# prismformore/Multi-Task-Transformer

Measured on AMD Instinct MI355X. Metric: training images/sec (512x512, 6 tasks), higher is better.
Workload: dtype f32(bf16x3)

## Files before the change

multi-task-transformer_amd/csrc/attn_fast.hip:

```cpp
#include "mtt_device.h"
#include <type_traits>

namespace {

constexpr int KV = 64, HD = 64;
constexpr int KTILE = KV * HD * 2;
constexpr float LOG2E = 1.4426950408889634f;

struct AttnP { mtt_attn_desc d; };

__device__ __attribute__((aligned(32))) const unsigned g_attn_zero_page[8] = {0u, 0u, 0u, 0u, 0u, 0u, 0u, 0u};
MTT_DEV void attn_glds16(const bf16_t* src, unsigned char* lds_wave_base) {
  __builtin_amdgcn_global_load_lds((const __attribute__((address_space(1))) void*)src,
                                   (__attribute__((address_space(3))) void*)lds_wave_base, 16, 0, 0);
}
MTT_DEV bool attn_block_dead(const mtt_attn_desc& d, int b, int qb) {
  return d.skip_scale != nullptr && qb * 128 >= d.T && d.skip_scale[2 * b + 1] == 0.0f;
}
MTT_DEV void attn_store_dead_block(const mtt_attn_desc& d, int b, int h, int qb) {
  const int N = d.N, C = d.nH * HD, tid = threadIdx.x;
  const u32x4 z = (u32x4){0u, 0u, 0u, 0u};
#pragma unroll
  for (int i = 0; i < 4; ++i) {
    const int idx = tid + 256 * i, qrow = qb * 128 + (idx >> 3);
    if (qrow >= N) continue;
    const int64_t oi = ((int64_t)b * N + qrow) * C + h * HD + (idx & 7) * 8;
    *(u32x4*)((bf16_t*)d.out + oi) = z;
    if (d.out_lo) *(u32x4*)((bf16_t*)d.out_lo + oi) = z;
  }
  if (d.lse && tid < 128 && qb * 128 + tid < N) d.lse[((int64_t)b * d.nH + h) * N + qb * 128 + tid] = 0.f;
}
template <int OFF>
MTT_DEV u32x2 attn_ds_read_tr16(unsigned addr) {
  u32x2 r;
  asm volatile("ds_read_b64_tr_b16 %0, %1 offset:%2" : "=v"(r) : "v"(addr), "n"(OFF) : "memory");
  return r;
}
__global__ __launch_bounds__(256, 2) void attn_fwd_fast_kernel(const AttnP p) {
  extern __shared__ __attribute__((aligned(16))) unsigned char smem[];
  constexpr int STAGE = 2 * KTILE;
  const mtt_attn_desc& d = p.d;
  const int nqb = (d.N + 127) / 128;
  const int wi = xcd_remap(blockIdx.x, gridDim.x);
  const int qb = wi % nqb, bh = wi / nqb;
  const int h = bh % d.nH, b = bh / d.nH;
  if (attn_block_dead(d, b, qb)) { attn_store_dead_block(d, b, h, qb); return; }
  const int N = d.N, C = d.nH * HD;
  const int tid = threadIdx.x, lane = tid & 63, wave = tid >> 6;
  const int li = lane & 15, lg = lane >> 4;
  const int64_t tok0 = (int64_t)b * N;
  const bf16_t* qkv = (const bf16_t*)d.qkv;
  const int q0 = qb * 128 + wave * 32;
  const bool active = q0 < N;

  u32x4 qf[2][2], dummy;
#pragma unroll
  for (int sub = 0; sub < 2; ++sub) {
    const int qrow = q0 + sub * 16 + li;
    const bool ok = qrow < N;
#pragma unroll
    for (int kh = 0; kh < 2; ++kh) {
      Raw8<false> r;
// ... 186 lines not shown
    if (qrow >= N) continue;
    const float inv = 1.0f / l;
#pragma unroll
    for (int dt = 0; dt < 4; ++dt)
      *(u32x2*)(out + (tok0 + qrow) * C + h * HD + dt * 16 + lg * 4) =
          (u32x2){pack2(o[sub][dt][0] * inv, o[sub][dt][1] * inv), pack2(o[sub][dt][2] * inv, o[sub][dt][3] * inv)};
    if (d.lse && lg == 0) d.lse[((int64_t)b * d.nH + h) * N + qrow] = (m_run[sub] + log2f(l)) * 0.6931471805599453f;
  }
}


__global__ __launch_bounds__(256, 2) void attn_fwd_x3_kernel(const AttnP p) {
  extern __shared__ __attribute__((aligned(16))) unsigned char smem[];
  constexpr int STAGE = 4 * KTILE;
  const mtt_attn_desc& d = p.d;
  const int nqb = (d.N + 127) / 128;
  const int wi = xcd_remap(blockIdx.x, gridDim.x);
  const int qb = wi % nqb, bh = wi / nqb;
  const int h = bh % d.nH, b = bh / d.nH;
  if (attn_block_dead(d, b, qb)) { attn_store_dead_block(d, b, h, qb); return; }
  const int N = d.N, C = d.nH * HD;
  const int tid = threadIdx.x, lane = tid & 63, wave = tid >> 6;
  const int li = lane & 15, lg = lane >> 4;
  const int64_t tok0 = (int64_t)b * N;
  const bf16_t* qh_ = (const bf16_t*)d.qkv;
  const bf16_t* ql_ = (const bf16_t*)d.qkv_lo;
  const int q0 = qb * 128 + wave * 32;
  const bool active = q0 < N;

  u32x4 qfh[2][2], qfl[2][2];
#pragma unroll
  for (int sub = 0; sub < 2; ++sub) {
    const int qrow = q0 + sub * 16 + li;
    const bool ok = qrow < N;
    const int64_t qi = (tok0 + (ok ? qrow : 0)) * 3 * C + h * HD + lg * 8;
#pragma unroll
    for (int kh = 0; kh < 2; ++kh) {
      const u32x4 z = (u32x4){0u, 0u, 0u, 0u};
      qfh[sub][kh] = ok ? *(const u32x4*)(qh_ + qi + kh * 32) : z;
      qfl[sub][kh] = ok ? *(const u32x4*)(ql_ + qi + kh * 32) : z;
    }
  }

  int dma_off[4], dma_row[2];
  uint64_t zpage = (uint64_t)(uintptr_t)g_attn_zero_page;
  asm volatile("" : "+s"(zpage));
#pragma unroll
  for (int i = 0; i < 2; ++i) {
    const int r = wave * 16 + i * 8 + (lane >> 3), pc = lane & 7;
    dma_row[i] = r;
    dma_off[i] = r * 3 * C + C + ((pc ^ (r >> 1)) & 7) * 8;
    dma_off[2 + i] = r * 3 * C + 2 * C + (((((pc >> 1) ^ (r >> 1)) & 3) << 1) | (pc & 1)) * 8;
  }
  auto dma_issue = [&](unsigned char* st, int kv0) {
    const int64_t boff = (tok0 + kv0) * 3 * C + h * HD;
    const bool full = kv0 + KV <= N;
#pragma unroll
    for (int pl = 0; pl < 2; ++pl) {
      const bf16_t* base = (pl ? ql_ : qh_) + boff;
#pragma unroll
      for (int kv = 0; kv < 2; ++kv) {
        unsigned char* dst = st + (kv * 2 + pl) * KTILE + wave * 2048;
#pragma unroll
        for (int i = 0; i < 2; ++i) {
          const bool ok = full || kv0 + dma_row[i] < N;
          attn_glds16((const bf16_t*)(uintptr_t)(ok ? (uint64_t)(uintptr_t)(base + dma_off[kv * 2 + i]) : zpage), dst + i * 1024);
        }
      }
    }
  };
  const int vrow = 4 * lg + (li >> 2);
  const int vf_ = (vrow >> 1) & 3;
  unsigned vaddr[4];
#pragma unroll
  for (int dt = 0; dt < 4; ++dt) vaddr[dt] = (unsigned)(uintptr_t)smem + (unsigned)(2 * KTILE + vrow * 128 + (li & 3) * 8 + ((dt ^ vf_) & 3) * 32);
  const unsigned char* kaddr[2];
#pragma unroll
  for (int kh = 0; kh < 2; ++kh) kaddr[kh] = smem + li * 128 + (((kh * 4 + lg) ^ (li >> 1)) & 7) * 16;

  f32x4 o[2][4];
#pragma unroll
  for (int sub = 0; sub < 2; ++sub)
#pragma unroll
    for (int t = 0; t < 4; ++t) o[sub][t] = (f32x4){0.f, 0.f, 0.f, 0.f};
  float m_run[2] = {-INFINITY, -INFINITY}, l_part[2] = {0.f, 0.f};
  const float sc2 = d.scale * LOG2E;
  const bool write_raw = d.rawlog != nullptr && d.T > 0 && qb == 0 && wave == 0 && li < d.T;

  const int nkv = (N + KV - 1) / KV;
  dma_issue(smem, 0);
  asm volatile("s_waitcnt vmcnt(0)" ::: "memory");
  __syncthreads();

  auto tile = [&](auto stage_tag, int j) {
    constexpr int ST = decltype(stage_tag)::value;
    const bool more = j + 1 < nkv;
    if (more) dma_issue(smem + (1 - ST) * STAGE, (j + 1) * KV);
    const int kv0 = j * KV;
    if (active) {
      f32x4 s[2][4];
      {
        u32x4 kf[4][2];
#pragma unroll
        for (int kt = 0; kt < 4; ++kt)
#pragma unroll
          for (int kh = 0; kh < 2; ++kh) kf[kt][kh] = *(const u32x4*)(kaddr[kh] + ST * STAGE + kt * 2048);
        __builtin_amdgcn_s_setprio(1);
#pragma unroll
        for (int kt = 0; kt < 4; ++kt) {
          s[0][kt] = (f32x4){0.f, 0.f, 0.f, 0.f};
          s[1][kt] = (f32x4){0.f, 0.f, 0.f, 0.f};
#pragma unroll
          for (int kh = 0; kh < 2; ++kh) {
            s[0][kt] = mfma16(kf[kt][kh], qfl[0][kh], s[0][kt]);
            s[1][kt] = mfma16(kf[kt][kh], qfl[1][kh], s[1][kt]);
            s[0][kt] = mfma16(kf[kt][kh], qfh[0][kh], s[0][kt]);
            s[1][kt] = mfma16(kf[kt][kh], qfh[1][kh], s[1][kt]);
          }
        }
        __builtin_amdgcn_s_setprio(0);
#pragma unroll
        for (int kt = 0; kt < 4; ++kt)
#pragma unroll
          for (int kh = 0; kh < 2; ++kh) kf[kt][kh] = *(const u32x4*)(kaddr[kh] + ST * STAGE + KTILE + kt * 2048);
        __builtin_amdgcn_s_setprio(1);
#pragma unroll
        for (int kt = 0; kt < 4; ++kt)
#pragma unroll
          for (int kh = 0; kh < 2; ++kh) {
            s[0][kt] = mfma16(kf[kt][kh], qfh[0][kh], s[0][kt]);
            s[1][kt] = mfma16(kf[kt][kh], qfh[1][kh], s[1][kt]);
          }
        __builtin_amdgcn_s_setprio(0);
      }
      if (write_raw) {
        float* rl = d.rawlog + (((int64_t)b * d.nH + h) * d.T + li) * N;
#pragma unroll
        for (int kt = 0; kt < 4; ++kt)
#pragma unroll
          for (int r = 0; r < 4; ++r) {
            const int key = kv0 + kt * 16 + lg * 4 + r;
            if (key < N) rl[key] = s[0][kt][r];
          }
      }
      if (kv0 + KV > N) {
#pragma unroll
        for (int sub = 0; sub < 2; ++sub)
#pragma unroll
          for (int kt = 0; kt < 4; ++kt)
#pragma unroll
            for (int r = 0; r < 4; ++r)
              if ((kv0 + kt * 16 + lg * 4 + r) >= N) s[sub][kt][r] = -INFINITY;
      }
      u32x4 pbh[2][2], pbl[2][2];
#pragma unroll
      for (int sub = 0; sub < 2; ++sub) {
        float mx = s[sub][0][0];
#pragma unroll
        for (int kt = 0; kt < 4; ++kt)
#pragma unroll
          for (int r = 0; r < 4; ++r) mx = fmaxf(mx, s[sub][kt][r]);
        mx = groups_max(mx);
        const float m_new = fmaxf(m_run[sub], mx * sc2);
        if (__builtin_amdgcn_ballot_w64(m_new != m_run[sub]) != 0) {
          const float alpha = __builtin_amdgcn_exp2f(m_run[sub] - m_new);
          l_part[sub] *= alpha;
#pragma unroll
          for (int t = 0; t < 4; ++t)
#pragma unroll
            for (int r = 0; r < 4; ++r) o[sub][t][r] *= alpha;
          m_run[sub] = m_new;
        }
        float rs = 0.f;
#pragma unroll
        for (int kt = 0; kt < 4; ++kt)
#pragma unroll
          for (int r = 0; r < 4; ++r) {
            const float pv = __builtin_amdgcn_exp2f(fmaf(s[sub][kt][r], sc2, -m_new));
            s[sub][kt][r] = pv;
            rs += pv;
          }
        l_part[sub] += rs;
#pragma unroll
        for (int ks = 0; ks < 2; ++ks) {
          const u32x4 ph = (u32x4){pack2(s[sub][2 * ks][0], s[sub][2 * ks][1]), pack2(s[sub][2 * ks][2], s[sub][2 * ks][3]),
                                   pack2(s[sub][2 * ks + 1][0], s[sub][2 * ks + 1][1]), pack2(s[sub][2 * ks + 1][2], s[sub][2 * ks + 1][3])};
          pbh[sub][ks] = ph;
          pbl[sub][ks] = (u32x4){pack2(s[sub][2 * ks][0] - lo_of(ph.x), s[sub][2 * ks][1] - hi_of(ph.x)),
                                 pack2(s[sub][2 * ks][2] - lo_of(ph.y), s[sub][2 * ks][3] - hi_of(ph.y)),
                                 pack2(s[sub][2 * ks + 1][0] - lo_of(ph.z), s[sub][2 * ks + 1][1] - hi_of(ph.z)),
                                 pack2(s[sub][2 * ks + 1][2] - lo_of(ph.w), s[sub][2 * ks + 1][3] - hi_of(ph.w))};
        }
      }
      const bool half1 = kv0 + 32 < N;
#define ATW(x) "+v"(x)
#pragma unroll
      for (int pass = 0; pass < 2; ++pass) {
        u32x2 v0l[4], v0h[4], v1l[4], v1h[4];
#pragma unroll
        for (int dt = 0; dt < 4; ++dt) {
          if (pass == 0) {
            v0l[dt] = attn_ds_read_tr16<ST * STAGE>(vaddr[dt]);
            v0h[dt] = attn_ds_read_tr16<ST * STAGE + 16 * 128>(vaddr[dt]);
          } else {
            v0l[dt] = attn_ds_read_tr16<ST * STAGE + KTILE>(vaddr[dt]);
            v0h[dt] = attn_ds_read_tr16<ST * STAGE + KTILE + 16 * 128>(vaddr[dt]);
          }
        }
#pragma unroll
        for (int dt = 0; dt < 4; ++dt) {
          if (pass == 0) {
            v1l[dt] = attn_ds_read_tr16<ST * STAGE + 32 * 128>(vaddr[dt]);
            v1h[dt] = attn_ds_read_tr16<ST * STAGE + 48 * 128>(vaddr[dt]);
          } else {
            v1l[dt] = attn_ds_read_tr16<ST * STAGE + KTILE + 32 * 128>(vaddr[dt]);
            v1h[dt] = attn_ds_read_tr16<ST * STAGE + KTILE + 48 * 128>(vaddr[dt]);
          }
        }
        asm volatile("s_waitcnt lgkmcnt(8)"
                     : ATW(v0l[0]), ATW(v0l[1]), ATW(v0l[2]), ATW(v0l[3]), ATW(v0h[0]), ATW(v0h[1]), ATW(v0h[2]), ATW(v0h[3]),
                       ATW(v1l[0]), ATW(v1l[1]), ATW(v1l[2]), ATW(v1l[3]), ATW(v1h[0]), ATW(v1h[1]), ATW(v1h[2]), ATW(v1h[3]) :: "memory");
        __builtin_amdgcn_s_setprio(1);
#pragma unroll
        for (int dt = 0; dt < 4; ++dt) {
          const u32x4 vf = (u32x4){v0l[dt][0], v0l[dt][1], v0h[dt][0], v0h[dt][1]};
          if (pass == 0) {
            o[0][dt] = mfma16(vf, pbl[0][0], o[0][dt]);
            o[1][dt] = mfma16(vf, pbl[1][0], o[1][dt]);
          }
          o[0][dt] = mfma16(vf, pbh[0][0], o[0][dt]);
          o[1][dt] = mfma16(vf, pbh[1][0], o[1][dt]);
        }
        asm volatile("s_waitcnt lgkmcnt(0)" : ATW(v1l[0]), ATW(v1l[1]), ATW(v1l[2]), ATW(v1l[3]), ATW(v1h[0]), ATW(v1h[1]), ATW(v1h[2]), ATW(v1h[3]) :: "memory");
        if (half1) {
#pragma unroll
          for (int dt = 0; dt < 4; ++dt) {
            const u32x4 vf = (u32x4){v1l[dt][0], v1l[dt][1], v1h[dt][0], v1h[dt][1]};
            if (pass == 0) {
              o[0][dt] = mfma16(vf, pbl[0][1], o[0][dt]);
              o[1][dt] = mfma16(vf, pbl[1][1], o[1][dt]);
            }
            o[0][dt] = mfma16(vf, pbh[0][1], o[0][dt]);
            o[1][dt] = mfma16(vf, pbh[1][1], o[1][dt]);
          }
        }
        __builtin_amdgcn_s_setprio(0);
      }
#undef ATW
    }
    if (more) asm volatile("s_waitcnt vmcnt(0)" ::: "memory");
    __syncthreads();
  };
  for (int j = 0; j < nkv; j += 2) {
    tile(std::integral_constant<int, 0>{}, j);
    if (j + 1 < nkv) tile(std::integral_constant<int, 1>{}, j + 1);
  }

  bf16_t* outh = (bf16_t*)d.out;
  bf16_t* outl = (bf16_t*)d.out_lo;
#pragma unroll
  for (int sub = 0; sub < 2; ++sub) {
    const float l = groups_sum(l_part[sub]);
    const int qrow = q0 + sub * 16 + li;
    if (qrow >= N) continue;
    const float inv = 1.0f / l;
#pragma unroll
    for (int dt = 0; dt < 4; ++dt) {
      const float v0 = o[sub][dt][0] * inv, v1 = o[sub][dt][1] * inv, v2 = o[sub][dt][2] * inv, v3 = o[sub][dt][3] * inv;
      const u32x2 hi = (u32x2){pack2(v0, v1), pack2(v2, v3)};
      const int64_t oi = (tok0 + qrow) * C + h * HD + dt * 16 + lg * 4;
      *(u32x2*)(outh + oi) = hi;
      *(u32x2*)(outl + oi) = (u32x2){pack2(v0 - lo_of(hi.x), v1 - hi_of(hi.x)), pack2(v2 - lo_of(hi.y), v3 - hi_of(hi.y))};
    }
    if (d.lse && lg == 0) d.lse[((int64_t)b * d.nH + h) * N + qrow] = (m_run[sub] + log2f(l)) * 0.6931471805599453f;
  }
}

}

int mtt_attn_fwd_x3_split(const mtt_attn_desc* dd, hipStream_t s) {
  constexpr int smem = 2 * 4 * KTILE;
  static std::atomic<unsigned long long> done{0};
  if (int e = mtt_ensure_dyn_lds((const void*)attn_fwd_x3_kernel, smem, done)) return e;
  AttnP p; p.d = *dd;
  dim3 grid((unsigned)(((dd->N + 127) / 128) * dd->nH * dd->B));
  hipLaunchKernelGGL(attn_fwd_x3_kernel, grid, dim3(256), smem, s, p);
  return (int)hipGetLastError();
}

int mtt_attn_fwd_fast(const mtt_attn_desc* dd, hipStream_t s) {
  constexpr int smem = 2 * 2 * KTILE;
  AttnP p; p.d = *dd;
  dim3 grid((unsigned)(((dd->N + 127) / 128) * dd->nH * dd->B));
  hipLaunchKernelGGL(attn_fwd_fast_kernel, grid, dim3(256), smem, s, p);
  return (int)hipGetLastError();
}
```

multi-task-transformer_amd/csrc/gemm.hip:

```cpp
#include "mtt_device.h"
#include <type_traits>

namespace {

#ifndef MTT_GROUP_M
#define MTT_GROUP_M 4
#endif
#ifndef MTT_RING
#define MTT_RING 1
#endif
constexpr int BM = 128, BN = 128, BK = 64;
constexpr int TILE_BYTES = BM * BK * 2;

struct GemmP {
  mtt_gemm_desc d;
  FastDiv divW, divH, divCp, div3;
  FastDiv divAmb, divDmb, divRmb;
  FastDiv divPsW, divPsH, divPsCo;
  FastDiv divSkip;
  int tiles_m, tiles_n;
  int group_m;
#ifdef MTT_GEMM_TRACE
  unsigned long long* trace;
#endif
};

#ifdef MTT_GEMM_TRACE
MTT_DEV unsigned long long trace_hwid() {
  unsigned a, b;
  asm volatile("s_getreg_b32 %0, hwreg(HW_REG_HW_ID)" : "=s"(a));
  asm volatile("s_getreg_b32 %0, hwreg(HW_REG_XCC_ID)" : "=s"(b));
  return (unsigned long long)a | ((unsigned long long)b << 32);
}
#define MTT_TRACE(slot) do { if (p.trace && threadIdx.x == 0) p.trace[(size_t)(blockIdx.x + gridDim.x * blockIdx.z) * 8 + (slot)] = __builtin_amdgcn_s_memtime(); } while (0)
#define MTT_TRACE_RT(slot) do { if (p.trace && threadIdx.x == 0) p.trace[(size_t)(blockIdx.x + gridDim.x * blockIdx.z) * 8 + (slot)] = __builtin_amdgcn_s_memrealtime(); } while (0)
#define MTT_TRACE_ID(tile) do { if (p.trace && threadIdx.x == 0) { p.trace[(size_t)(blockIdx.x + gridDim.x * blockIdx.z) * 8 + 6] = trace_hwid(); p.trace[(size_t)(blockIdx.x + gridDim.x * blockIdx.z) * 8 + 7] = (tile); } } while (0)
#else
#define MTT_TRACE(slot) do {} while (0)
#define MTT_TRACE_RT(slot) do {} while (0)
#define MTT_TRACE_ID(tile) do {} while (0)
#endif

MTT_DEV int64_t row_off(uint32_t m, int mb, int64_t bs, int64_t ld, FastDiv f) {
  if (mb <= 0) return (int64_t)m * ld;
  const uint32_t q = fdiv(m, f);
  return (int64_t)q * bs + (int64_t)(m - q * (uint32_t)mb) * ld;
}

MTT_DEV bool skip_rows_dead(const GemmP& p, uint32_t r0, uint32_t r1) {
  const uint32_t mb = (uint32_t)p.d.skip_mb, np = (uint32_t)p.d.skip_prompt;
  uint32_t q = fdiv(r0, p.divSkip);
  uint32_t o = r0 - q * mb;
  for (uint32_t r = r0; r < r1;) {
    const uint32_t c = o >= np ? 1u : 0u;
    if (p.d.skip_scale[2 * q + c] != 0.0f) return false;
    if (c) { r += mb - o; ++q; o = 0; }
    else { r += np - o; o = np; if (np == mb) { ++q; o = 0; } }
  }
  return true;
}


__device__ __attribute__((aligned(32))) const unsigned g_zero_page[8] = {0u, 0u, 0u, 0u, 0u, 0u, 0u, 0u};

template <bool X3, bool CONV, bool F32>
struct StagerK {
  const void* base; int dtype; int K; int c;
  int64_t roff[4]; bool rok[4];
  uint64_t zpage;
  unsigned tapmask[4];
  int tap, ci, knext;
  Raw8<F32> raw[4];

  MTT_DEV void init(const GemmP& p, const void* b, int dt, int row0, int rows, int64_t ld, int mb, int64_t bs, FastDiv fmb) {
// ... 1443 lines not shown

  for (int kt = 0; kt < nk; ++kt) {
    const unsigned st = (unsigned)((kt & 1) * STAGE);
#pragma unroll
    for (int kh = 0; kh < 2; ++kh) {
      if (kh == 0 && kt + 1 < nk) issue((kt + 1) & 1, kt + 1);
      const unsigned off = st + (unsigned)(kh * 32 * 512);
      u32x2 bl[NT], bh[NT], al[MT], ah[MT];
#pragma unroll
      for (int t = 0; t < NT; ++t) { bl[t] = ds_read_tr16(b_addr[t] + off); bh[t] = ds_read_tr16(b_addr[t] + off + 4 * 512); }
#pragma unroll
      for (int t = 0; t < MT; ++t) { al[t] = ds_read_tr16(a_addr[t] + off); ah[t] = ds_read_tr16(a_addr[t] + off + 4 * 512); }
#define TNW(x) "+v"(x)
#define TNW_A TNW(al[0]), TNW(al[1]), TNW(al[2]), TNW(al[3]), TNW(al[4]), TNW(al[5]), TNW(al[6]), TNW(al[7]), \
              TNW(ah[0]), TNW(ah[1]), TNW(ah[2]), TNW(ah[3]), TNW(ah[4]), TNW(ah[5]), TNW(ah[6]), TNW(ah[7])
      if constexpr (MEDGE) {
        if (kh == 1) asm volatile("s_waitcnt vmcnt(0) lgkmcnt(0)" : TNW(bl[0]), TNW(bl[1]), TNW(bh[0]), TNW(bh[1]), TNW_A :: "memory");
        else asm volatile("s_waitcnt lgkmcnt(0)" : TNW(bl[0]), TNW(bl[1]), TNW(bh[0]), TNW(bh[1]), TNW_A :: "memory");
      } else {
        if (kh == 1)
          asm volatile("s_waitcnt vmcnt(0) lgkmcnt(0)"
                       : TNW(bl[0]), TNW(bl[1]), TNW(bl[2]), TNW(bl[3]), TNW(bh[0]), TNW(bh[1]), TNW(bh[2]), TNW(bh[3]), TNW_A :: "memory");
        else
          asm volatile("s_waitcnt lgkmcnt(0)"
                       : TNW(bl[0]), TNW(bl[1]), TNW(bl[2]), TNW(bl[3]), TNW(bh[0]), TNW(bh[1]), TNW(bh[2]), TNW(bh[3]), TNW_A :: "memory");
      }
#undef TNW_A
#undef TNW
      u32x4 fa[MT], fb[NT];
#pragma unroll
      for (int t = 0; t < NT; ++t) fb[t] = (u32x4){bl[t][0], bl[t][1], bh[t][0], bh[t][1]};
#pragma unroll
      for (int t = 0; t < MT; ++t) fa[t] = (u32x4){al[t][0], al[t][1], ah[t][0], ah[t][1]};
      __builtin_amdgcn_sched_barrier(0);
      __builtin_amdgcn_s_barrier();
      __builtin_amdgcn_sched_barrier(0);
      __builtin_amdgcn_s_setprio(1);
#pragma unroll
      for (int a = 0; a < MT; ++a)
#pragma unroll
        for (int b = 0; b < NT; ++b) acc[a][b] = mfma16(fa[a], fb[b], acc[a][b]);
      __builtin_amdgcn_s_setprio(0);
      __builtin_amdgcn_sched_barrier(0);
      __builtin_amdgcn_s_barrier();
      __builtin_amdgcn_sched_barrier(0);
    }
  }
  if (!late) __builtin_amdgcn_s_barrier();
  __syncthreads();
  if constexpr (MEDGE) gemm_epilogue<256, WAVES_M, WAVES_N, MT, NT>(p, acc, smem, m0, n0, zo, zi);
  else gemm_epilogue_auto<256, WAVES_M, WAVES_N, MT, NT>(p, acc, smem, m0, n0, zo, zi);
}

template <bool CONVB>
__global__ __launch_bounds__(512, 1) void gemm_tn_kernel(const GemmP p) {
  extern __shared__ __attribute__((aligned(16))) unsigned char smem[];
  const int wg = xcd_remap(blockIdx.x, gridDim.x);
  const int tiles_n = (p.d.N + 255) / 256, tiles_m = (p.d.M + 255) / 256;
  int tile_m, tile_n;
  grouped_tile(wg, tiles_m, tiles_n, p.group_m, tile_m, tile_n);
  const int m0 = tile_m * 256, n0 = tile_n * 256;
  const int z = blockIdx.z;
  const int zo = z / p.d.batch_inner, zi = z - zo * p.d.batch_inner;
  if (MTT_R3_EDGE && p.d.M - m0 <= 128 && !p.d.colsum_out && p.d.store_mode == MTT_STORE_ROWS) tn_tile<CONVB, true>(p, smem, m0, n0, zo, zi);
  else tn_tile<CONVB, false>(p, smem, m0, n0, zo, zi);
}

template <bool CONVB>
int launch_tn(const GemmP& p, hipStream_t stream) {
  constexpr int smem = 2 * 2 * BK * 256 * 2;
  static std::atomic<unsigned long long> done{0};
  if (int e = mtt_ensure_dyn_lds((const void*)gemm_tn_kernel<CONVB>, smem, done)) return e;
  const int tm = (p.d.M + 255) / 256, tn = (p.d.N + 255) / 256;
  dim3 grid(tm * tn, 1, p.d.batch);
  hipLaunchKernelGGL((gemm_tn_kernel<CONVB>), grid, dim3(512), smem, stream, p);
  return (int)hipGetLastError();
}

FastDiv make_div(uint32_t dv) {
  FastDiv f; f.d = dv ? dv : 1u;
  uint32_t s = 0; while ((1ull << s) < f.d) ++s;
  f.shift = s;
  f.magic = (uint32_t)((((1ull << 32) * ((1ull << s) - f.d)) / f.d) + 1ull);
  return f;
}

template <int AOP, int BOP, int MODE>
int launch(const GemmP& p, hipStream_t stream) {
  constexpr int smem = TILE_BYTES * 2 * (MODE == 2 ? 2 : 1) * 2;
  static std::atomic<unsigned long long> done{0};
  if (int e = mtt_ensure_dyn_lds((const void*)gemm_kernel<AOP, BOP, MODE>, smem, done)) return e;
  dim3 grid(p.tiles_m * p.tiles_n, 1, p.d.batch);
  hipLaunchKernelGGL((gemm_kernel<AOP, BOP, MODE>), grid, dim3(256), smem, stream, p);
  return (int)hipGetLastError();
}

}

extern "C" int mtt_abi_version(void) { return MTT_ABI_VERSION; }

extern "C" size_t mtt_desc_size(int which) {
  switch (which) {
    case 0: return sizeof(mtt_gemm_desc);
    case 1: return sizeof(mtt_attn_desc);
    case 2: return sizeof(mtt_softmax_desc);
    case 3: return sizeof(mtt_ln_desc);
    case 4: return sizeof(mtt_chanlogit_desc);
    case 5: return sizeof(mtt_modulate_desc);
    case 6: return sizeof(mtt_ctr_desc);
    case 7: return sizeof(mtt_resize_desc);
    case 8: return sizeof(mtt_bn_desc);
    case 9: return sizeof(mtt_conv_geom);
    case 10: return sizeof(mtt_dwconv_desc);
    case 11: return sizeof(mtt_pool_desc);
    case 12: return sizeof(mtt_lnmt_desc);
    case 13: return sizeof(mtt_attnmsg_desc);
    case 14: return sizeof(mtt_convt_desc);
    case 15: return sizeof(mtt_adam_desc);
// ... 12 lines not shown

static bool dma_fastaddr_ok(const mtt_gemm_desc& d, int kmod = 64) {
  if (d.K % kmod) return false;
  const int64_t a_span = (d.a_mb > 0 ? (int64_t)((d.M - 1) / d.a_mb) * d.a_bs + (int64_t)((d.M - 1) % d.a_mb) * d.lda : (int64_t)(d.M - 1) * d.lda) + d.K;
  const int64_t b_span = (int64_t)(d.N - 1) * d.ldb + d.K;
  return a_span < (1ll << 31) && b_span < (1ll << 31);
}
static int gemm_variant_for(const mtt_gemm_desc& d) {
  const bool any_split = d.a_dtype == MTT_SPLIT || d.b_dtype == MTT_SPLIT;
  if (any_split) {
    const bool both = d.prec == MTT_PREC_X3 && d.a_dtype == MTT_SPLIT && d.b_dtype == MTT_SPLIT && d.b_op == MTT_OP_K && d.A_lo && d.B_lo &&
                      d.store_mode == MTT_STORE_ROWS;
    if (d.a_scale) return MTT_E_UNSUPPORTED;
    if (both && d.a_op == MTT_OP_K && dma_fastaddr_ok(d, MTT_RING ? 32 : 64) && d.K >= 64 && d.K / 64 * 3 < 32768) return 8;
    if (both && d.a_op == MTT_OP_CONV_K && d.conv.Cp % 32 == 0 && d.conv.Cp <= 4096 && d.K == 9 * d.conv.Cp && d.a_mb <= 0 &&
        (int64_t)d.M * d.lda < (1ll << 31) && (int64_t)(d.N - 1) * d.ldb + d.K < (1ll << 31)) return 9;
    return MTT_E_UNSUPPORTED;
  }
  if (f32n_ok(d)) return 11;
  if (d.a_scale) return MTT_E_UNSUPPORTED;
  if (d.prec != MTT_PREC_BF16 || d.a_dtype != MTT_BF16 || d.b_dtype != MTT_BF16) return 0;
  if (d.a_op == MTT_OP_CONV_K && d.b_op == MTT_OP_K && d.variant != MTT_GEMM_GENERAL && d.store_mode == MTT_STORE_ROWS && d.conv.Cp % 32 == 0 &&
      d.conv.Cp <= 4096 && d.K == 9 * d.conv.Cp && d.lda == d.conv.Cp && d.a_mb <= 0 && (int64_t)d.M * d.lda < (1ll << 31) &&
      (int64_t)(d.N - 1) * d.ldb + d.K < (1ll << 31) && !d.colsum_out &&
      (d.variant == MTT_GEMM_DMA256 || (d.M >= 2048 && d.N >= 128))) return 12;
  const bool tn = d.a_op == MTT_OP_R && (d.b_op == MTT_OP_R || d.b_op == MTT_OP_CONV_R) && d.store_mode == MTT_STORE_ROWS;
  if (tn && d.variant != MTT_GEMM_GENERAL) {
    if (d.variant == MTT_GEMM_DMA256) return 6;
    const int64_t pm = (d.M + 255) / 256 * 256, pn = (d.N + 255) / 256 * 256;
    const int batch = d.batch < 1 ? 1 : d.batch;
    const bool fills = (pm / 256) * (pn / 256) * batch >= 64 && d.K >= 512;
    if (fills && 100 * (int64_t)d.M * d.N >= 45 * pm * pn) return 6;
    return 0;
  }
  const bool dma = d.a_op == MTT_OP_K && d.b_op == MTT_OP_K && (d.K % 8) == 0;
  if (!dma || d.variant == MTT_GEMM_GENERAL) return 0;
  if (d.variant == MTT_GEMM_DMA256) return 3;
  if (d.variant == MTT_GEMM_DMA128) return 4;
  const int n256 = (d.N + 255) / 256 * 256, n128 = (d.N + 127) / 128 * 128;
  const bool wide = 100 * n128 > 85 * n256;
  const int batch = d.batch < 1 ? 1 : d.batch;
  const int64_t blocks = (int64_t)((d.M + 255) / 256) * ((d.N + 255) / 256) * batch;
  if (wide && d.M >= 512 && d.N >= 512 && blocks >= 96) return 3;
  const int tbn = 32 * dma128_nt(d);
  const int64_t blocks128 = (int64_t)((d.M + 127) / 128) * ((d.N + tbn - 1) / tbn) * batch;
  if (d.M >= 512 && d.K >= 128 && blocks128 >= 256) return 4;
  if (d.M >= 128 && d.N >= 256 && d.K >= 512) return 4;
  return 0;
}
#ifdef MTT_GEMM_TRACE
static unsigned long long* g_trace_host = nullptr;
extern "C" void mtt_debug_set_trace(void* buf) { g_trace_host = (unsigned long long*)buf; }
#endif
extern "C" int mtt_gemm_variant(const mtt_gemm_desc* d) { return d ? gemm_variant_for(*d) : MTT_E_BADARG; }

static int gemm_launch(GemmP& p, hipStream_t s, int v);
extern "C" int mtt_gemm(const mtt_gemm_desc* dd, void* stream) {
  if (!dd || !dd->A || !dd->B || !dd->D) return MTT_E_BADARG;
  GemmP p; p.d = *dd;
  mtt_gemm_desc& d = p.d;
  if (d.M <= 0 || d.N <= 0 || d.K <= 0) return MTT_E_BADARG;
  if (d.batch < 1) d.batch = 1;
  if (d.batch_inner < 1) d.batch_inner = 1;
  const bool a_k = d.a_op == MTT_OP_K || d.a_op == MTT_OP_CONV_K, b_k = d.b_op == MTT_OP_K;
  const int Kp8 = (d.K + 7) / 8 * 8;
  if ((a_k && d.a_op == MTT_OP_K && d.lda < Kp8) || (b_k && d.ldb < Kp8)) return MTT_E_ALIGN;
  if (d.a_op == MTT_OP_CONV_K && (d.K % 8)) return MTT_E_ALIGN;
  if ((d.lda % 8) || (d.ldb % 8)) return MTT_E_ALIGN;
  if (((uintptr_t)d.A & 15) || ((uintptr_t)d.B & 15)) return MTT_E_ALIGN;
  if ((d.aux_in || d.aux_out) && (d.ldaux <= 0 || (d.ldaux % 8))) return MTT_E_BADARG;
  if (d.act < MTT_ACT_NONE || d.act > MTT_ACT_MUL_AUX) return MTT_E_BADARG;
  if ((d.act == MTT_ACT_GELU_DAUX && !d.aux_out) || ((d.act == MTT_ACT_MUL_AUX || d.act == MTT_ACT_GELU_BWD || d.act == MTT_ACT_RELU_BWD) && !d.aux_in))
    return MTT_E_BADARG;
  if ((d.ldd % 8) || ((uintptr_t)d.D & 15) || (d.d_bs % 8) || (d.d_zo % 8) || (d.d_zi % 8)) return MTT_E_ALIGN;
  if (d.resid && ((d.ldr % 4) || ((uintptr_t)d.resid & 15) || (d.r_bs % 4))) return MTT_E_ALIGN;
  const bool conv = d.a_op == MTT_OP_CONV_K || d.b_op == MTT_OP_CONV_R;
  if (conv) {
    if (d.conv.H <= 0 || d.conv.W <= 0 || d.conv.Cp % 8 || d.conv.C > d.conv.Cp || d.conv.dil < 1) return MTT_E_BADARG;
    if (d.a_op == MTT_OP_CONV_K && d.K != 9 * d.conv.Cp) return MTT_E_BADARG;
    if (d.b_op == MTT_OP_CONV_R && d.N != 9 * d.conv.Cp) return MTT_E_BADARG;
  }
  if (d.store_mode == MTT_STORE_PIXSHUF2 && (d.ps_H <= 0 || d.ps_W <= 0 || d.ps_Co <= 0 || d.N != 4 * d.ps_Co)) return MTT_E_BADARG;
  p.divW = make_div(conv ? d.conv.W : 1); p.divH = make_div(conv ? d.conv.H : 1);
  p.divCp = make_div(conv ? d.conv.Cp : 1); p.div3 = make_div(3);
  p.divAmb = make_div(d.a_mb > 0 ? d.a_mb : 1); p.divDmb = make_div(d.d_mb > 0 ? d.d_mb : 1);
  p.divRmb = make_div(d.r_mb > 0 ? d.r_mb : 1);
  p.divPsW = make_div(d.ps_W > 0 ? d.ps_W : 1); p.divPsH = make_div(d.ps_H > 0 ? d.ps_H : 1);
  p.divPsCo = make_div(d.ps_Co > 0 ? d.ps_Co : 1);
  if (d.skip_scale) {
    if (d.skip_mb <= 0 || d.skip_prompt < 0 || d.skip_prompt > d.skip_mb || d.skip_row0 < 0) return MTT_E_BADARG;
  }
  p.divSkip = make_div(d.skip_scale ? d.skip_mb : 1);
  p.tiles_m = (d.M + BM - 1) / BM; p.tiles_n = (d.N + BN - 1) / BN;
  p.group_m = MTT_GROUP_M;
#ifdef MTT_GEMM_TRACE
  p.trace = g_trace_host;
#endif
  hipStream_t s = (hipStream_t)stream;
  const int v = gemm_variant_for(d);
  if (v < 0) return v;
  if (d.d_dtype == MTT_SPLIT && !d.D_lo) return MTT_E_BADARG;
  if (d.d_dtype == MTT_SPLIT && d.store_mode != MTT_STORE_ROWS) return MTT_E_UNSUPPORTED;
  if (d.colsum_out) {
    if (!d.colsum_ws) return MTT_E_BADARG;
    if (d.batch != 1 || d.store_mode != MTT_STORE_ROWS || v == 6) return MTT_E_UNSUPPORTED;
    const int rc = gemm_launch(p, s, v);
    if (rc) return rc;
    const int tbm = (v == 3 || v == 8 || v == 9) ? 256 : BM;
    hipLaunchKernelGGL(mtt_colsum_final_kernel, dim3((d.N + 31) / 32, 1, 1), dim3(256), 0, s, (const float*)d.colsum_ws, d.colsum_out, d.N,
                       (d.M + tbm - 1) / tbm, (int64_t)0);
    return (int)hipGetLastError();
  }
  return gemm_launch(p, s, v);
}

extern "C" size_t mtt_gemm_colsum_ws_floats(const mtt_gemm_desc* d) {
  if (!d || d->M <= 0 || d->N <= 0) return 0;
  return (size_t)((d->M + BM - 1) / BM) * (size_t)((d->N + 7) / 8 * 8);
}

static int gemm_launch(GemmP& p, hipStream_t s, int v) {
  mtt_gemm_desc& d = p.d;
  if (v == 11) return launch_f32n(p, s);
  if (v == 12) return launch_ringc(p, s);
  if (v == 9) return launch_ring3<true>(p, s);
#if MTT_RING
  if (v == 8) return launch_ring3<false>(p, s);
#else
  if (v == 8) return launch_dma<2>(p, s);
#endif
  if (v == 3) return dma_fastaddr_ok(d) ? launch_dma<1>(p, s) : launch_dma<0>(p, s);
  if (v == 4) {
    const bool fa = dma_fastaddr_ok(d);
    switch (dma128_nt(d)) {
      case 1: return fa ? launch_dma128<true, 1>(p, s) : launch_dma128<false, 1>(p, s);
      case 2: return fa ? launch_dma128<true, 2>(p, s) : launch_dma128<false, 2>(p, s);
      default: return fa ? launch_dma128<true, 4>(p, s) : launch_dma128<false, 4>(p, s);
    }
  }
  if (v == 6) return d.b_op == MTT_OP_CONV_R ? launch_tn<true>(p, s) : launch_tn<false>(p, s);
  int mode;
  if (d.prec == MTT_PREC_X3) {
    if (d.a_dtype != MTT_F32 || d.b_dtype != MTT_F32) return MTT_E_UNSUPPORTED;
    mode = 2;
  } else if (d.a_dtype == MTT_BF16 && d.b_dtype == MTT_BF16) mode = 0;
  else if (d.a_dtype == MTT_F32 && d.b_dtype == MTT_BF16) mode = 1;
  else if (d.a_dtype == MTT_F32 && d.b_dtype == MTT_F32) { mode = 3; if (d.colsum_out) return MTT_E_UNSUPPORTED; }
// ... 14 lines not shown
```

multi-task-transformer_amd/csrc/mtt_device.h:

```cpp
#pragma once
#include <hip/hip_runtime.h>
#include <stdint.h>
#include <atomic>
#include "mtt_hip.h"

static inline int mtt_ensure_dyn_lds(const void* fn, int bytes, std::atomic<unsigned long long>& done) {
  int dev = 0;
  if (hipGetDevice(&dev) != hipSuccess) return (int)hipGetLastError();
  const unsigned long long bit = 1ull << (dev & 63);
  if (done.load(std::memory_order_acquire) & bit) return 0;
  const hipError_t e = hipFuncSetAttribute(fn, hipFuncAttributeMaxDynamicSharedMemorySize, bytes);
  if (e != hipSuccess) return (int)e;
  done.fetch_or(bit, std::memory_order_release);
  return 0;
}

typedef unsigned short bf16_t;
typedef __attribute__((ext_vector_type(8))) __bf16 bf16x8;
typedef __attribute__((ext_vector_type(4))) float f32x4;
typedef __attribute__((ext_vector_type(4))) unsigned int u32x4;
typedef __attribute__((ext_vector_type(2))) unsigned int u32x2;

#define MTT_DEV __device__ __forceinline__

MTT_DEV float bf2f(bf16_t h) { return __builtin_bit_cast(float, ((unsigned)h) << 16); }
MTT_DEV bf16_t f2bf(float f) { return __builtin_bit_cast(bf16_t, (__bf16)f); }
typedef __attribute__((ext_vector_type(2))) float f32x2_t;
typedef __attribute__((ext_vector_type(2))) __bf16 bf16x2_t;
MTT_DEV unsigned pack2(float a, float b) {
  return __builtin_bit_cast(unsigned, __builtin_convertvector((f32x2_t){a, b}, bf16x2_t));
}
MTT_DEV float lo_of(unsigned u) { return __builtin_bit_cast(float, u << 16); }
MTT_DEV float hi_of(unsigned u) { return __builtin_bit_cast(float, u & 0xffff0000u); }

MTT_DEV float ld_elem(const void* p, int64_t idx, int dtype) {
  return dtype == MTT_F32 ? ((const float*)p)[idx] : bf2f(((const bf16_t*)p)[idx]);
}
MTT_DEV void st_elem(void* p, int64_t idx, int dtype, float v) {
  if (dtype == MTT_F32) ((float*)p)[idx] = v; else ((bf16_t*)p)[idx] = f2bf(v);
}

MTT_DEV float fast_erf(float x) {
  x = fminf(fmaxf(x, -4.0f), 4.0f);
  const float x2 = x * x;
  float p = fmaf(x2, -2.72614225801306e-10f, 2.77068142495902e-08f);
  p = fmaf(x2, p, -2.10102402082508e-06f);
  p = fmaf(x2, p, -5.69250639462346e-05f);
  p = fmaf(x2, p, -7.34990630326855e-04f);
  p = fmaf(x2, p, -2.95459980854025e-03f);
  p = fmaf(x2, p, -1.60960333262415e-02f);
  float q = fmaf(x2, -1.45660718464996e-05f, -2.13374055278905e-04f);
  q = fmaf(x2, q, -1.68282697438203e-03f);
  q = fmaf(x2, q, -7.37332916720468e-03f);
  q = fmaf(x2, q, -1.42647390514189e-02f);
  return x * p * __builtin_amdgcn_rcpf(q);
}
MTT_DEV float gelu_f(float x) { return 0.5f * x * (1.0f + fast_erf(x * 0.70710678118654752f)); }
MTT_DEV void gelu_both_f(float x, float& g, float& dg) {
  const float c = 0.5f * (1.0f + fast_erf(x * 0.70710678118654752f));
  g = x * c;
  dg = fmaf(x * 0.3989422804014327f, __expf(-0.5f * x * x), c);
}
MTT_DEV float gelu_grad_f(float x) {
  return 0.5f * (1.0f + fast_erf(x * 0.70710678118654752f)) + x * 0.3989422804014327f * __expf(-0.5f * x * x);
}

MTT_DEV int lds_swz(int row) { return ((row >> 1) ^ (row >> 4)) & 7; }
MTT_DEV int lds_off(int row, int chunk) { return row * 128 + (((chunk ^ lds_swz(row)) & 7) << 4); }

struct FastDiv { uint32_t magic, shift, d; };
MTT_DEV uint32_t fdiv(uint32_t n, FastDiv f) { return (__umulhi(n, f.magic) + n) >> f.shift; }

template <bool X3>
MTT_DEV void load8(const void* base, int64_t idx, int dtype, bool ok, u32x4& hi, u32x4& lo) {
  hi = (u32x4){0u, 0u, 0u, 0u};
  if (X3) lo = hi;
// ... 154 lines not shown
```

Before: 185.3.

## Specialize full KV tiles and one-subtile path in attention; add fast TN GEMM issue

The attention forward kernel gains compile-time specialized tile variants. Full KV tiles use a cheaper DMA issue with a uniform scalar base pointer and precomputed 32-bit offsets, and skip the bounds masking. Edge query blocks with a single valid 16-row subtile skip the second subtile's MFMAs and softmax. A new tn_tile_fast path for interior TN GEMM tiles issues global-to-LDS loads with scalar base pointers that step each iteration, instead of recomputing a 64-bit address per lane with bounds checks. This adds code size and register pressure, and both paths sit behind environment switches that default to on.

```diff
diff --git a/multi-task-transformer_amd/csrc/attn_fast.hip b/multi-task-transformer_amd/csrc/attn_fast.hip
--- a/multi-task-transformer_amd/csrc/attn_fast.hip
+++ b/multi-task-transformer_amd/csrc/attn_fast.hip
@@ -7,7 +7,11 @@
 constexpr int KTILE = KV * HD * 2;
 constexpr float LOG2E = 1.4426950408889634f;
 
-struct AttnP { mtt_attn_desc d; };
+struct AttnP { mtt_attn_desc d; int flags; };
+constexpr int AFWD_TILES = 1, AFWD_ONESUB = 2;
+using Tag0 = std::integral_constant<int, 0>;
+using Tag1 = std::integral_constant<int, 1>;
+using Tag2 = std::integral_constant<int, 2>;
 
 __device__ __attribute__((aligned(32))) const unsigned g_attn_zero_page[8] = {0u, 0u, 0u, 0u, 0u, 0u, 0u, 0u};
 MTT_DEV void attn_glds16(const bf16_t* src, unsigned char* lds_wave_base) {
@@ -300,6 +304,24 @@
     dma_off[i] = r * 3 * C + C + ((pc ^ (r >> 1)) & 7) * 8;
     dma_off[2 + i] = r * 3 * C + 2 * C + (((((pc >> 1) ^ (r >> 1)) & 3) << 1) | (pc & 1)) * 8;
   }
+  uint32_t dma_boff[4];
+#pragma unroll
+  for (int i = 0; i < 4; ++i) dma_boff[i] = (uint32_t)dma_off[i] * 2u;
+  const size_t kvoff0 = (size_t)(tok0 * 3 * C + h * HD) * 2;
+  const size_t kvstep = (size_t)KV * 3 * C * 2;
+  auto dma_issue_full = [&](unsigned char* st, int jt) {
+    const size_t boff = kvoff0 + (size_t)jt * kvstep;
+#pragma unroll
+    for (int pl = 0; pl < 2; ++pl) {
+      const unsigned char* base = uniform_ptr((const unsigned char*)(pl ? ql_ : qh_) + boff);
+#pragma unroll
+      for (int kv = 0; kv < 2; ++kv) {
+        unsigned char* dst = st + (kv * 2 + pl) * KTILE + wave * 2048;
+#pragma unroll
+        for (int i = 0; i < 2; ++i) attn_glds16((const bf16_t*)(base + opaque32(dma_boff[kv * 2 + i])), dst + i * 1024);
+      }
+    }
+  };
   auto dma_issue = [&](unsigned char* st, int kv0) {
     const int64_t boff = (tok0 + kv0) * 3 * C + h * HD;
     const bool full = kv0 + KV <= N;
@@ -335,15 +357,18 @@
   const float sc2 = d.scale * LOG2E;
   const bool write_raw = d.rawlog != nullptr && d.T > 0 && qb == 0 && wave == 0 && li < d.T;
 
-  const int nkv = (N + KV - 1) / KV;
-  dma_issue(smem, 0);
+  const int nkv = (N + KV - 1) / KV, nfull = N / KV;
+  const bool tiles = (p.flags & AFWD_TILES) != 0;
+  if (tiles && nfull > 0) dma_issue_full(smem, 0); else dma_issue(smem, 0);
   asm volatile("s_waitcnt vmcnt(0)" ::: "memory");
   __syncthreads();
 
-  auto tile = [&](auto stage_tag, int j) {
-    constexpr int ST = decltype(stage_tag)::value;
-    const bool more = j + 1 < nkv;
-    if (more) dma_issue(smem + (1 - ST) * STAGE, (j + 1) * KV);
+  auto tile = [&](auto stage_tag, auto kind_tag, auto nsub_tag, int j) __attribute__((always_inline)) {
+    constexpr int ST = decltype(stage_tag)::value, KIND = decltype(kind_tag)::value, NSUB = decltype(nsub_tag)::value;
+    constexpr bool FULL = KIND >= 1;
+    const bool more = KIND == 2 || j + 1 < nkv;
+    if constexpr (KIND == 2) dma_issue_full(smem + (1 - ST) * STAGE, j + 1);
+    else if (more) dma_issue(smem + (1 - ST) * STAGE, (j + 1) * KV);
     const int kv0 = j * KV;
     if (active) {
       f32x4 s[2][4];
@@ -357,13 +382,13 @@
 #pragma unroll
         for (int kt = 0; kt < 4; ++kt) {
           s[0][kt] = (f32x4){0.f, 0.f, 0.f, 0.f};
-          s[1][kt] = (f32x4){0.f, 0.f, 0.f, 0.f};
+          if (NSUB == 2) s[1][kt] = (f32x4){0.f, 0.f, 0.f, 0.f};
 #pragma unroll
           for (int kh = 0; kh < 2; ++kh) {
             s[0][kt] = mfma16(kf[kt][kh], qfl[0][kh], s[0][kt]);
-            s[1][kt] = mfma16(kf[kt][kh], qfl[1][kh], s[1][kt]);
+            if (NSUB == 2) s[1][kt] = mfma16(kf[kt][kh], qfl[1][kh], s[1][kt]);
             s[0][kt] = mfma16(kf[kt][kh], qfh[0][kh], s[0][kt]);
-            s[1][kt] = mfma16(kf[kt][kh], qfh[1][kh], s[1][kt]);
+            if (NSUB == 2) s[1][kt] = mfma16(kf[kt][kh], qfh[1][kh], s[1][kt]);
           }
         }
         __builtin_amdgcn_s_setprio(0);
@@ -377,7 +402,7 @@
 #pragma unroll
           for (int kh = 0; kh < 2; ++kh) {
             s[0][kt] = mfma16(kf[kt][kh], qfh[0][kh], s[0][kt]);
-            s[1][kt] = mfma16(kf[kt][kh], qfh[1][kh], s[1][kt]);
+            if (NSUB == 2) s[1][kt] = mfma16(kf[kt][kh], qfh[1][kh], s[1][kt]);
           }
         __builtin_amdgcn_s_setprio(0);
       }
@@ -388,12 +413,12 @@
 #pragma unroll
           for (int r = 0; r < 4; ++r) {
             const int key = kv0 + kt * 16 + lg * 4 + r;
-            if (key < N) rl[key] = s[0][kt][r];
-          }
-      }
-      if (kv0 + KV > N) {
-#pragma unroll
-        for (int sub = 0; sub < 2; ++sub)
+            if (FULL || key < N) rl[key] = s[0][kt][r];
+          }
+      }
+      if (!FULL && kv0 + KV > N) {
+#pragma unroll
+        for (int sub = 0; sub < NSUB; ++sub)
 #pragma unroll
           for (int kt = 0; kt < 4; ++kt)
 #pragma unroll
@@ -402,7 +427,7 @@
       }
       u32x4 pbh[2][2], pbl[2][2];
 #pragma unroll
-      for (int sub = 0; sub < 2; ++sub) {
+      for (int sub = 0; sub < NSUB; ++sub) {
         float mx = s[sub][0][0];
 #pragma unroll
         for (int kt = 0; kt < 4; ++kt)
@@ -440,7 +465,7 @@
                                  pack2(s[sub][2 * ks + 1][2] - lo_of(ph.w), s[sub][2 * ks + 1][3] - hi_of(ph.w))};
         }
       }
-      const bool half1 = kv0 + 32 < N;
+      const bool half1 = FULL || kv0 + 32 < N;
 #define ATW(x) "+v"(x)
 #pragma unroll
       for (int pass = 0; pass < 2; ++pass) {
@@ -474,10 +499,10 @@
           const u32x4 vf = (u32x4){v0l[dt][0], v0l[dt][1], v0h[dt][0], v0h[dt][1]};
           if (pass == 0) {
             o[0][dt] = mfma16(vf, pbl[0][0], o[0][dt]);
-            o[1][dt] = mfma16(vf, pbl[1][0], o[1][dt]);
+            if (NSUB == 2) o[1][dt] = mfma16(vf, pbl[1][0], o[1][dt]);
           }
           o[0][dt] = mfma16(vf, pbh[0][0], o[0][dt]);
-          o[1][dt] = mfma16(vf, pbh[1][0], o[1][dt]);
+          if (NSUB == 2) o[1][dt] = mfma16(vf, pbh[1][0], o[1][dt]);
         }
         asm volatile("s_waitcnt lgkmcnt(0)" : ATW(v1l[0]), ATW(v1l[1]), ATW(v1l[2]), ATW(v1l[3]), ATW(v1h[0]), ATW(v1h[1]), ATW(v1h[2]), ATW(v1h[3]) :: "memory");
         if (half1) {
@@ -486,10 +511,10 @@
             const u32x4 vf = (u32x4){v1l[dt][0], v1l[dt][1], v1h[dt][0], v1h[dt][1]};
             if (pass == 0) {
               o[0][dt] = mfma16(vf, pbl[0][1], o[0][dt]);
-              o[1][dt] = mfma16(vf, pbl[1][1], o[1][dt]);
+              if (NSUB == 2) o[1][dt] = mfma16(vf, pbl[1][1], o[1][dt]);
             }
             o[0][dt] = mfma16(vf, pbh[0][1], o[0][dt]);
-            o[1][dt] = mfma16(vf, pbh[1][1], o[1][dt]);
+            if (NSUB == 2) o[1][dt] = mfma16(vf, pbh[1][1], o[1][dt]);
           }
         }
         __builtin_amdgcn_s_setprio(0);
@@ -499,10 +524,30 @@
     if (more) asm volatile("s_waitcnt vmcnt(0)" ::: "memory");
     __syncthreads();
   };
-  for (int j = 0; j < nkv; j += 2) {
-    tile(std::integral_constant<int, 0>{}, j);
-    if (j + 1 < nkv) tile(std::integral_constant<int, 1>{}, j + 1);
-  }
+  auto run = [&](auto nsub) __attribute__((always_inline)) {
+    if (!tiles) {
+      for (int j = 0; j < nkv; j += 2) {
+        tile(Tag0{}, Tag0{}, nsub, j);
+        if (j + 1 < nkv) tile(Tag1{}, Tag0{}, nsub, j + 1);
+      }
+      return;
+    }
+    int j = 0;
+    for (; j + 2 < nfull; j += 2) {
+      tile(Tag0{}, Tag2{}, nsub, j);
+      tile(Tag1{}, Tag2{}, nsub, j + 1);
+    }
+    if (j + 1 < nfull) { tile(Tag0{}, Tag2{}, nsub, j); ++j; }
+    if (j < nfull) {
+      if (j & 1) tile(Tag1{}, Tag1{}, nsub, j); else tile(Tag0{}, Tag1{}, nsub, j);
+      ++j;
+    }
+    if (j < nkv) {
+      if (j & 1) tile(Tag1{}, Tag0{}, nsub, j); else tile(Tag0{}, Tag0{}, nsub, j);
+    }
+  };
+  const bool onesub = (p.flags & AFWD_ONESUB) != 0 && __builtin_amdgcn_readfirstlane((int)(q0 + 16 >= N)) != 0;
+  if (onesub) run(Tag1{}); else run(Tag2{});
 
   bf16_t* outh = (bf16_t*)d.out;
   bf16_t* outl = (bf16_t*)d.out_lo;
@@ -526,11 +571,13 @@
 
 }
 
+static const int g_afwd_flags = (mtt_env_switch("MTT_AFWD_TILES", 1) ? AFWD_TILES : 0) | (mtt_env_switch("MTT_AFWD_ONESUB", 1) ? AFWD_ONESUB : 0);
+
 int mtt_attn_fwd_x3_split(const mtt_attn_desc* dd, hipStream_t s) {
   constexpr int smem = 2 * 4 * KTILE;
   static std::atomic<unsigned long long> done{0};
   if (int e = mtt_ensure_dyn_lds((const void*)attn_fwd_x3_kernel, smem, done)) return e;
-  AttnP p; p.d = *dd;
+  AttnP p; p.d = *dd; p.flags = g_afwd_flags;
   dim3 grid((unsigned)(((dd->N + 127) / 128) * dd->nH * dd->B));
   hipLaunchKernelGGL(attn_fwd_x3_kernel, grid, dim3(256), smem, s, p);
   return (int)hipGetLastError();
@@ -538,7 +585,7 @@
 
 int mtt_attn_fwd_fast(const mtt_attn_desc* dd, hipStream_t s) {
   constexpr int smem = 2 * 2 * KTILE;
-  AttnP p; p.d = *dd;
+  AttnP p; p.d = *dd; p.flags = 0;
   dim3 grid((unsigned)(((dd->N + 127) / 128) * dd->nH * dd->B));
   hipLaunchKernelGGL(attn_fwd_fast_kernel, grid, dim3(256), smem, s, p);
   return (int)hipGetLastError();
diff --git a/multi-task-transformer_amd/csrc/gemm.hip b/multi-task-transformer_amd/csrc/gemm.hip
--- a/multi-task-transformer_amd/csrc/gemm.hip
+++ b/multi-task-transformer_amd/csrc/gemm.hip
@@ -20,6 +20,7 @@
   FastDiv divSkip;
   int tiles_m, tiles_n;
   int group_m;
+  int tn_fast;
 #ifdef MTT_GEMM_TRACE
   unsigned long long* trace;
 #endif
@@ -1569,6 +1570,139 @@
   else gemm_epilogue_auto<256, WAVES_M, WAVES_N, MT, NT>(p, acc, smem, m0, n0, zo, zi);
 }
 
+MTT_DEV void tn_tile_fast(const GemmP& p, unsigned char* smem, int m0, int n0, int zo, int zi) {
+  constexpr int MT = 8, NT = 4, WAVES_N = 4, WAVES_M = 2;
+  constexpr int TILE = BK * 256 * 2, STAGE = 2 * TILE;
+  const bf16_t* Abase = (const bf16_t*)p.d.A + ((int64_t)zo * p.d.a_zo + (int64_t)zi * p.d.a_zi);
+  const bf16_t* Bbase = (const bf16_t*)p.d.B + ((int64_t)zo * p.d.b_zo + (int64_t)zi * p.d.b_zi);
+  const int lane = threadIdx.x & 63, wave = __builtin_amdgcn_readfirstlane(threadIdx.x >> 6);
+  const int wm = wave >> 2, wn = wave & 3;
+  const int late = wave >> 2;
+  const int K = p.d.K;
+  uint64_t zpage = (uint64_t)(uintptr_t)g_zero_page;
+  asm volatile("" : "+s"(zpage));
+
+  const int c16 = lane & 31, unitp = c16 >> 1, hb = c16 & 1;
+  int fk[4];
+#pragma unroll
+  for (int i = 0; i < 4; ++i) {
+    const int k = wave * 8 + 2 * i + (lane >> 5);
+    fk[i] = (k & 3) | (((k >> 3) & 1) << 2);
+  }
+  auto src_col = [&](int i) { return (((unitp & 8) | ((unitp & 7) ^ fk[i])) * 2 + hb) * 8; };
+  const unsigned char* Ak = uniform_ptr((const unsigned char*)(Abase + ((int64_t)(wave * 8) * p.d.lda + m0)));
+  const unsigned char* Bk = uniform_ptr((const unsigned char*)(Bbase + ((int64_t)(wave * 8) * p.d.ldb + n0)));
+  const size_t a_step = (size_t)p.d.lda * (BK * 2), b_step = (size_t)p.d.ldb * (BK * 2);
+  uint32_t aoff32[4], boff32[4];
+#pragma unroll
+  for (int i = 0; i < 4; ++i) {
+    aoff32[i] = (uint32_t)((lane >> 5) + 2 * i) * (uint32_t)p.d.lda * 2u + (uint32_t)src_col(i) * 2u;
+    boff32[i] = (uint32_t)((lane >> 5) + 2 * i) * (uint32_t)p.d.ldb * 2u + (uint32_t)src_col(i) * 2u;
+  }
+  auto issue_fast = [&](int stage) {
+    unsigned char* sA = smem + stage * STAGE + wave * 4096;
+    const unsigned char* a = uniform_ptr(Ak);
+#pragma unroll
+    for (int i = 0; i < 4; ++i) glds16((const bf16_t*)(a + opaque32(aoff32[i])), sA + i * 1024);
+    Ak += a_step;
+    const unsigned char* b = uniform_ptr(Bk);
+#pragma unroll
+    for (int i = 0; i < 4; ++i) glds16((const bf16_t*)(b + opaque32(boff32[i])), sA + TILE + i * 1024);
+    Bk += b_step;
+  };
+  auto issue_ragged = [&](int stage, int kt) {
+    unsigned char* sA = smem + stage * STAGE + wave * 4096;
+    const int k0 = kt * BK + wave * 8 + (lane >> 5);
+#pragma unroll
+    for (int i = 0; i < 4; ++i) {
+      const int k = k0 + 2 * i;
+      const uint64_t srca = (uint64_t)(uintptr_t)(Abase + ((int64_t)k * p.d.lda + (m0 + src_col(i))));
+      glds16((const bf16_t*)(uintptr_t)(k < K ? srca : zpage), sA + i * 1024);
+    }
+#pragma unroll
+    for (int i = 0; i < 4; ++i) {
+      const int k = k0 + 2 * i;
+      const uint64_t srcb = (uint64_t)(uintptr_t)(Bbase + ((int64_t)k * p.d.ldb + (n0 + src_col(i))));
+      glds16((const bf16_t*)(uintptr_t)(k < K ? srcb : zpage), sA + TILE + i * 1024);
+    }
+  };
+
+  const int r16 = lane & 15, g = lane >> 4;
+  const int fr = (r16 >> 2) | ((g & 1) << 2);
+  const unsigned lbase = (unsigned)(uintptr_t)smem + (unsigned)((8 * g + (r16 >> 2)) * 512 + (r16 & 3) * 8);
+  unsigned a_addr[MT], b_addr[NT];
+#pragma unroll
+  for (int t = 0; t < MT; ++t) a_addr[t] = lbase + (unsigned)((wm * 8 + (t ^ fr)) * 32);
+#pragma unroll
+  for (int t = 0; t < NT; ++t) {
+    const int unit = wn * NT + t;
+    b_addr[t] = lbase + (unsigned)TILE + (unsigned)(((unit & 8) | ((unit & 7) ^ fr)) * 32);
+  }
+
+  f32x4 acc[MT][NT];
+#pragma unroll
+  for (int a = 0; a < MT; ++a)
+#pragma unroll
+    for (int b = 0; b < NT; ++b) acc[a][b] = (f32x4){0.f, 0.f, 0.f, 0.f};
+
+  const int nk = (K + BK - 1) / BK, nfull = K / BK;
+  issue_fast(0);
+  asm volatile("s_waitcnt vmcnt(0)" ::: "memory");
+  __builtin_amdgcn_s_barrier();
+  if (late) __builtin_amdgcn_s_barrier();
+  __builtin_amdgcn_sched_barrier(0);
+
+  auto kstep = [&](int kt, auto next_tag) __attribute__((always_inline)) {
+    constexpr int NEXT = decltype(next_tag)::value;
+    const unsigned st = (unsigned)((kt & 1) * STAGE);
+#pragma unroll
+    for (int kh = 0; kh < 2; ++kh) {
+      if (kh == 0) {
+        if constexpr (NEXT == 2) issue_fast((kt + 1) & 1);
+        if constexpr (NEXT == 1) { if (kt + 1 < nk) issue_ragged((kt + 1) & 1, kt + 1); }
+      }
+      const unsigned off = st + (unsigned)(kh * 32 * 512);
+      u32x2 bl[NT], bh[NT], al[MT], ah[MT];
+#pragma unroll
+      for (int t = 0; t < NT; ++t) { bl[t] = ds_read_tr16(b_addr[t] + off); bh[t] = ds_read_tr16(b_addr[t] + off + 4 * 512); }
+#pragma unroll
+      for (int t = 0; t < MT; ++t) { al[t] = ds_read_tr16(a_addr[t] + off); ah[t] = ds_read_tr16(a_addr[t] + off + 4 * 512); }
+#define TNW(x) "+v"(x)
+#define TNW_AB TNW(bl[0]), TNW(bl[1]), TNW(bl[2]), TNW(bl[3]), TNW(bh[0]), TNW(bh[1]), TNW(bh[2]), TNW(bh[3]), \
+               TNW(al[0]), TNW(al[1]), TNW(al[2]), TNW(al[3]), TNW(al[4]), TNW(al[5]), TNW(al[6]), TNW(al[7]), \
+               TNW(ah[0]), TNW(ah[1]), TNW(ah[2]), TNW(ah[3]), TNW(ah[4]), TNW(ah[5]), TNW(ah[6]), TNW(ah[7])
+      if (kh == 1) asm volatile("s_waitcnt vmcnt(0) lgkmcnt(0)" : TNW_AB :: "memory");
+      else asm volatile("s_waitcnt lgkmcnt(0)" : TNW_AB :: "memory");
+#undef TNW_AB
+#undef TNW
+      u32x4 fa[MT], fb[NT];
+#pragma unroll
+      for (int t = 0; t < NT; ++t) fb[t] = (u32x4){bl[t][0], bl[t][1], bh[t][0], bh[t][1]};
+#pragma unroll
+      for (int t = 0; t < MT; ++t) fa[t] = (u32x4){al[t][0], al[t][1], ah[t][0], ah[t][1]};
+      __builtin_amdgcn_sched_barrier(0);
+      __builtin_amdgcn_s_barrier();
+      __builtin_amdgcn_sched_barrier(0);
+      __builtin_amdgcn_s_setprio(1);
+#pragma unroll
+      for (int a = 0; a < MT; ++a)
+#pragma unroll
+        for (int b = 0; b < NT; ++b) acc[a][b] = mfma16(fa[a], fb[b], acc[a][b]);
+      __builtin_amdgcn_s_setprio(0);
+      __builtin_amdgcn_sched_barrier(0);
+      __builtin_amdgcn_s_barrier();
+      __builtin_amdgcn_sched_barrier(0);
+    }
+  };
+  int kt = 0;
+  for (; kt + 1 < nfull; ++kt) kstep(kt, std::integral_constant<int, 2>{});
+  kstep(kt, std::integral_constant<int, 1>{});
+  if (nk > nfull) kstep(kt + 1, std::integral_constant<int, 0>{});
+  if (!late) __builtin_amdgcn_s_barrier();
+  __syncthreads();
+  gemm_epilogue_auto<256, WAVES_M, WAVES_N, MT, NT>(p, acc, smem, m0, n0, zo, zi);
+}
+
 template <bool CONVB>
 __global__ __launch_bounds__(512, 1) void gemm_tn_kernel(const GemmP p) {
   extern __shared__ __attribute__((aligned(16))) unsigned char smem[];
@@ -1579,8 +1713,15 @@
   const int m0 = tile_m * 256, n0 = tile_n * 256;
   const int z = blockIdx.z;
   const int zo = z / p.d.batch_inner, zi = z - zo * p.d.batch_inner;
-  if (MTT_R3_EDGE && p.d.M - m0 <= 128 && !p.d.colsum_out && p.d.store_mode == MTT_STORE_ROWS) tn_tile<CONVB, true>(p, smem, m0, n0, zo, zi);
-  else tn_tile<CONVB, false>(p, smem, m0, n0, zo, zi);
+  if (MTT_R3_EDGE && p.d.M - m0 <= 128 && !p.d.colsum_out && p.d.store_mode == MTT_STORE_ROWS) { tn_tile<CONVB, true>(p, smem, m0, n0, zo, zi); return; }
+  if constexpr (!CONVB) {
+    const int64_t ldmax = p.d.lda > p.d.ldb ? p.d.lda : p.d.ldb;
+    if (p.tn_fast && m0 + 256 <= p.d.M && n0 + 256 <= p.d.N && p.d.K >= BK && 8 * ldmax * 2 + 512 < (1ll << 32)) {
+      tn_tile_fast(p, smem, m0, n0, zo, zi);
+      return;
+    }
+  }
+  tn_tile<CONVB, false>(p, smem, m0, n0, zo, zi);
 }
 
 template <bool CONVB>
@@ -1699,6 +1840,7 @@
 static unsigned long long* g_trace_host = nullptr;
 extern "C" void mtt_debug_set_trace(void* buf) { g_trace_host = (unsigned long long*)buf; }
 #endif
+static const int g_tn_fastissue = mtt_env_switch("MTT_TN_FASTISSUE", 1);
 extern "C" int mtt_gemm_variant(const mtt_gemm_desc* d) { return d ? gemm_variant_for(*d) : MTT_E_BADARG; }
 
 static int gemm_launch(GemmP& p, hipStream_t s, int v);
@@ -1740,6 +1882,7 @@
   p.divSkip = make_div(d.skip_scale ? d.skip_mb : 1);
   p.tiles_m = (d.M + BM - 1) / BM; p.tiles_n = (d.N + BN - 1) / BN;
   p.group_m = MTT_GROUP_M;
+  p.tn_fast = g_tn_fastissue;
 #ifdef MTT_GEMM_TRACE
   p.trace = g_trace_host;
 #endif
diff --git a/multi-task-transformer_amd/csrc/mtt_device.h b/multi-task-transformer_amd/csrc/mtt_device.h
--- a/multi-task-transformer_amd/csrc/mtt_device.h
+++ b/multi-task-transformer_amd/csrc/mtt_device.h
@@ -1,6 +1,7 @@
 #pragma once
 #include <hip/hip_runtime.h>
 #include <stdint.h>
+#include <stdlib.h>
 #include <atomic>
 #include "mtt_hip.h"
 
@@ -15,6 +16,12 @@
   return 0;
 }
 
+static inline int mtt_env_switch(const char* name, int dflt) {
+  const char* v = getenv(name);
+  if (!v || (v[0] != '0' && v[0] != '1') || v[1] != '\0') return dflt;
+  return v[0] == '1';
+}
+
 typedef unsigned short bf16_t;
 typedef __attribute__((ext_vector_type(8))) __bf16 bf16x8;
 typedef __attribute__((ext_vector_type(4))) float f32x4;
@@ -22,6 +29,16 @@
 typedef __attribute__((ext_vector_type(2))) unsigned int u32x2;
 
 #define MTT_DEV __device__ __forceinline__
+
+MTT_DEV const unsigned char* uniform_ptr(const unsigned char* q) {
+  const uint64_t v = (uint64_t)(uintptr_t)q;
+  const uint32_t lo = (uint32_t)__builtin_amdgcn_readfirstlane((int)(uint32_t)v), hi = (uint32_t)__builtin_amdgcn_readfirstlane((int)(uint32_t)(v >> 32));
+  return (const unsigned char*)(uintptr_t)(((uint64_t)hi << 32) | lo);
+}
+MTT_DEV uint32_t opaque32(uint32_t v) {
+  asm volatile("" : "+v"(v));
+  return v;
+}
 
 MTT_DEV float bf2f(bf16_t h) { return __builtin_bit_cast(float, ((unsigned)h) << 16); }
 MTT_DEV bf16_t f2bf(float f) { return __builtin_bit_cast(bf16_t, (__bf16)f); }
```

Result: no change. 186.5 (median of 6 runs) (+0.7%).
